# proroklab/gnn_pathplanning

Measured on AMD Instinct MI355X. Metric: agent-steps/sec (policy fwd), higher is better.
Workload: dtype f32 (bf16x3 exact operand split, f32 accumulate); 1 GPU; policy forward (addGSO+forward), 10 agents, 20x20 map GSO, K=3, batch=512 per GPU, eval mode, fp32 GSO resident in HBM; the SAME resident batch every step (inputs are L2 / Infinity-Cache warm by construction); agents=10, taps=3, batch_per_gpu=512, global_batch=512, parallelism=replicas x1

## Files before the change

gnn_pathplanning_amd/_native.py:

```python
import ctypes
import os
import shutil
import subprocess

import torch

_HERE = os.path.dirname(os.path.abspath(__file__))
CSRC = os.path.join(_HERE, 'csrc')
LIB_PATH = os.path.join(_HERE, 'libgnnpp.so')
MEASURE_LIB_PATH = os.path.join(_HERE, 'libgnnpp_measure.so')
VALIDATED_HIPCC = 'HIP version: 7.2.26015-fc0010cf6a'
TOOLCHAIN_STAMP = LIB_PATH + '.toolchain'
H2_UNSAFE_MARK = LIB_PATH + '.split_f16_disabled'
HEADER = os.path.join(os.path.dirname(_HERE), 'include', 'gnnpp.h')
MAPF_DISTANCE_HEADER = os.path.join(os.path.dirname(_HERE), 'include', 'gnnpp_mapf_distance.h')
CASEGEN_HEADER = os.path.join(os.path.dirname(_HERE), 'include', 'gnnpp_casegen.h')
CASEGEN_MAZE_HEADER = os.path.join(os.path.dirname(_HERE), 'include', 'gnnpp_casegen_maze.h')
MAPF_AUDIT_HEADER = os.path.join(os.path.dirname(_HERE), 'include', 'gnnpp_mapf_audit.h')
ROLLOUT_TRACE_HEADER = os.path.join(os.path.dirname(_HERE), 'include', 'gnnpp_rollout_trace.h')
SCHEDULE_DRAW_HEADER = os.path.join(os.path.dirname(_HERE), 'include', 'gnnpp_schedule_draw.h')
ROLLOUT_STREAM_HEADER = os.path.join(os.path.dirname(_HERE), 'include', 'gnnpp_rollout_stream.h')
ROLLOUT_STREAM_TRACE_HEADER = os.path.join(os.path.dirname(_HERE), 'include', 'gnnpp_rollout_stream_trace.h')
HIPCC_FLAGS = ['--offload-arch=gfx950', '-O3', '-std=c++17', '-shared', '-fPIC',
               '-Wno-unused-result']


class GnnppError(RuntimeError):
    pass


OK, ERR_ARG, ERR_UNSUPPORTED, ERR_LAUNCH, ERR_RANGE = 0, -1, -2, -3, -4
PREC_FP32, PREC_FP32_MFMA, PREC_SPLIT_F16 = 0, 1, 2
OBS_C, OBS_HW, FEAT, ACTIONS = 3, 11, 128, 5
MAX_NODES, MAX_ROWS = 100, 112
TUNE_FILTER_GPW, TUNE_FILTER_WAVES, TUNE_FUSED_POLICY, TUNE_FILTER_SPLIT, TUNE_POLICY_FILTER = 1, 2, 6, 7, 9
TUNE_FILTER_SMALL, TUNE_FILTER_SMALL_ROWS, TUNE_FILTER_PIPE_GRID = 10, 11, 12
TUNE_POLICY_CP, TUNE_ENCODER_CP_TILE, TUNE_FILTER_PLANE_ALIAS = 13, 14, 16
TUNE_TRAIN_WGRAD_WGS, TUNE_TRAIN_RUNNING_FUSED, TUNE_ENCODER_ONE_PLANE = 17, 19, 20
ROLLOUT_MAX_AGENTS, ROLLOUT_MAX_TEAM, ROLLOUT_TEAM_MAX_CELLS = 128, 1024, 65536
TIE_LOWEST, TIE_HASHED, TIE_REPLAY, TIE_MT19937 = 0, 1, 2, 3
SCHEDULE_BAD_MOVE, SCHEDULE_BAD_STATE, SCHEDULE_NO_RADIUS = 1, 2, 4
MAPF_NO_PATH, MAPF_BAD_CASE = 1, 2
MAPF_MAX_SIDE, MAPF_MAX_STEPS, MAPF_TEAM_MAX_SIDE, MAPF_TEAM_MAX_STEPS = 64, 1024, 256, 2048
MAPF_DIST_UNREACHABLE, MAPF_DIST_INVALID = -1, -2
MAPF_ORDER_INDEX, MAPF_ORDER_LONGEST_FIRST, MAPF_ORDER_SHORTEST_FIRST, MAPF_ORDER_HASHED = 0, 1, 2, 3
CASEGEN_OK, CASEGEN_TOO_SMALL = 0, 1
MAPF_AUDIT_CHUNK = 32
MAPF_AUDIT_CLASS_STATE, MAPF_AUDIT_CLASS_VERTEX, MAPF_AUDIT_CLASS_MOVE, MAPF_AUDIT_CLASS_SWAP = 0, 1, 2, 3
MAPF_AUDIT_STATE, MAPF_AUDIT_VERTEX, MAPF_AUDIT_MOVE, MAPF_AUDIT_SWAP = 1, 2, 4, 8
MAPF_AUDIT_BAD_START, MAPF_AUDIT_NOT_AT_GOAL, MAPF_AUDIT_SKIPPED = 16, 32, 64
TUNE_FILTER_ABLATE, TUNE_ENCODER_STOP = 3, 4
TUNE_POLICY_CP_TEAM = 21
PRECISIONS = {'fp32': PREC_FP32, 'fp32_mfma': PREC_FP32_MFMA, 'split_f16': PREC_SPLIT_F16}


def precision_code(p):
    if isinstance(p, str):
        if p not in PRECISIONS:
            raise GnnppError('unknown precision %r (one of %s)' % (p, sorted(PRECISIONS)))
        p = PRECISIONS[p]
    else:
        p = int(p)
        if p not in (PREC_FP32, PREC_FP32_MFMA, PREC_SPLIT_F16):
            raise GnnppError('unknown precision code %d' % p)
    if p == PREC_SPLIT_F16 and os.path.exists(H2_UNSAFE_MARK):
        raise GnnppError("precision 'split_f16' is disabled in this build: the ISA hipcc generated for the opt-in "
                         "split-f16 encoder failed the weight-ring check (%s); the default 'fp32' and 'fp32_mfma' "
                         "are unaffected" % open(H2_UNSAFE_MARK).read().strip()[:200])
    return p


def _sources():
    return [os.path.join(CSRC, f) for f in sorted(os.listdir(CSRC))] + [HEADER, MAPF_DISTANCE_HEADER, CASEGEN_HEADER,
                                                                          MAPF_AUDIT_HEADER, ROLLOUT_TRACE_HEADER,
                                                                          SCHEDULE_DRAW_HEADER, ROLLOUT_STREAM_HEADER,
                                                                          CASEGEN_MAZE_HEADER, ROLLOUT_STREAM_TRACE_HEADER]


def build(force=False, verbose=False, measure=False):
    out = MEASURE_LIB_PATH if measure else LIB_PATH
    if (not force and os.path.exists(out)
            and os.path.getmtime(out) >= max(os.path.getmtime(s) for s in _sources())):
        return out
    hipcc = shutil.which('hipcc') or '/opt/rocm/bin/hipcc'
    if not os.path.exists(hipcc):
        raise GnnppError('hipcc not found: libgnnpp.so cannot be built on this machine')
    tmp = os.path.join(_HERE, 'build', 'measure' if measure else 'product')
    os.makedirs(tmp, exist_ok=True)
    tmp_lib = os.path.join(tmp, 'libgnnpp.so')
    cmd = [hipcc] + HIPCC_FLAGS + (['-DGNNPP_MEASURE'] if measure else []) + \
          ['-save-temps', os.path.join(CSRC, 'gnnpp_api.hip'), '-o', tmp_lib]
    if verbose:
        print(' '.join(cmd))
    subprocess.check_call(cmd, cwd=tmp)
    isa = os.path.join(tmp, 'gnnpp_api-hip-amdgcn-amd-amdhsa-gfx950.s')
    h2_errors = check_ring_isa(isa, verbose=verbose)
    if not measure:
        if h2_errors:
            with open(H2_UNSAFE_MARK, 'w') as f:
                f.write('; '.join(h2_errors))
        elif os.path.exists(H2_UNSAFE_MARK):
            os.remove(H2_UNSAFE_MARK)
    if not measure:
        try:
            ver = subprocess.check_output([hipcc, '--version'], stderr=subprocess.STDOUT).decode().splitlines()[0].strip()
        except (OSError, subprocess.CalledProcessError, IndexError):
            ver = 'unknown'
        with open(TOOLCHAIN_STAMP, 'w') as f:
            f.write(ver + '\n')
    for f in os.listdir(tmp):
        if f != os.path.basename(isa) and f != 'libgnnpp.so':
            os.remove(os.path.join(tmp, f))
    os.replace(tmp_lib, out)
    return out


RING_KERNELS = (('encoder_kernel_b3ILb0ELi3ELb0E', 294, 0), ('encoder_kernel_b3ILb1ELi2ELb0E', 342, 32),
                ('encoder_kernel_b3ILb1ELi3ELb0E', 366, 32), ('encoder_kernel_b3ILb1ELi4ELb0E', 390, 32),
                ('encoder_kernel_b3ILb1ELi2ELb1ELi0E', 342, 32), ('encoder_kernel_b3ILb1ELi3ELb1ELi0E', 366, 32),
                ('encoder_kernel_b3ILb1ELi4ELb1ELi0E', 390, 32), ('encoder_kernel_b3ILb0ELi3ELb1ELi0E', 294, 0))
RING_KERNELS_TEAM = (('encoder_kernel_b3ILb1ELi2ELb1ELi10E', 342, 32), ('encoder_kernel_b3ILb1ELi3ELb1ELi10E', 366, 32),
                     ('encoder_kernel_b3ILb1ELi4ELb1ELi10E', 390, 32))
RING_KERNELS_OPTIONAL = (('encoder_kernel_h2ILb0ELi3E', 196, 0), ('encoder_kernel_h2ILb1ELi2E', 228, 32),
                         ('encoder_kernel_h2ILb1ELi3E', 244, 32), ('encoder_kernel_h2ILb1ELi4E', 260, 32))


def check_ring_isa(isa_path, verbose=False):
    import importlib.util
    spec = importlib.util.spec_from_file_location(
        'gnnpp_check_ring_isa', os.path.join(os.path.dirname(_HERE), 'tools', 'check_ring_isa.py'))
    mod = importlib.util.module_from_spec(spec)
    spec.loader.exec_module(mod)
    optional_errors = []
    for kern, items, scratch in RING_KERNELS + RING_KERNELS_TEAM + RING_KERNELS_OPTIONAL:
        errors, stats, meta = mod.check(isa_path, kern, scratch)
# ... 467 lines not shown
```

gnn_pathplanning_amd/csrc/encoder_kernel_b3.hip:

```cpp
#include <utility>

#include "gnnpp_common.h"

namespace gnnpp {

constexpr int kb_L1 = 0, kb_L2 = 54, kb_L3 = 108, kb_L4 = 162, kb_FC = 270, kb_END = 294;
constexpr int kb_FILT = kb_END;

constexpr int kB3Frag = 1024;
constexpr int kB3Region = 25 * 3 * kB3Frag;
constexpr int kB3Obs2 = kObsFloatsLds * 4;
constexpr int kB3L2out = 0, kB3L3out = 24 * kB3Frag, kB3L4out = 48 * kB3Frag;
constexpr int kB3Table = kB3Region;
constexpr int kB3TableBytes = EncLayout::kBssFloats * 4 + 16;
constexpr int kB3TableBytesFused = 5120;
constexpr int kB3SsmOff = 776 * 4;
constexpr size_t kB3Smem = kB3Region + kB3TableBytes;
constexpr size_t kB3SmemFused = kB3Region + kB3TableBytesFused;
static_assert(2 * kObsFloatsLds * 4 <= kB3Region && kB3SsmOff + 16 * 17 * 4 <= kB3TableBytesFused &&
              2 * kB3SmemFused <= (size_t)kLdsBytes, "b3 LDS map");
constexpr int kPkChan = 73;
constexpr int kPkAgent = 231;
constexpr int kPkBytes = kTileAgents * kPkAgent * 4;
constexpr int kB3ForcePlanes = 256;
constexpr int kL0Held = 2;
static_assert(kPkChan >= kPadHW * kPadHW / 2 && kPkAgent >= 3 * kPkChan && (kPkAgent & 1) && kPkBytes % 16 == 0 &&
              kPkBytes <= 2 * kObsFloatsLds * 4, "packed pixel image");
constexpr int kB3ZBytes = 16 * kZs * 4;
constexpr int kB3PRow = 3 * 256 + 32;
constexpr int kB3PBytes = 16 * kB3PRow;
constexpr int kB3POff = 2 * kB3ZBytes;
static_assert(kB3POff + kPolicyTapsMax * kB3PBytes + 4 * 16 * 8 * 4 <= kB3Region, "fused tail fits R");
constexpr size_t policy_sim_occ_bytes_b3() {
    return (size_t)kB3POff - 8 * kMaxAgents * sizeof(int) - kGsoSmemBytes;
}

struct WStreamB {
    const float* seg[6];
    int lane_bytes;
};

__device__ __forceinline__ const float* ring_item_ptr(const WStreamB& ws, int idx) {
    if (idx < kb_L2) return ws.seg[0] + (idx - kb_L1) * EncLayout::kHItem;
    if (idx < kb_L3) return ws.seg[1] + (idx - kb_L2) * EncLayout::kHItem;
    if (idx < kb_L4) return ws.seg[2] + (idx - kb_L3) * EncLayout::kHItem;
    if (idx < kb_FC) return ws.seg[3] + (idx - kb_L4) * EncLayout::kHItem;
    if (idx < kb_FILT) return ws.seg[4] + (idx - kb_FC) * EncLayout::kHItem;
    const int j = idx - kb_FILT, pl = j % 3, ml = (j / 3) & 1, kb = (j / 6) & 3, tap = j / 24;
    return ws.seg[5] + tap * (8 * 4 * 768) + ml * (4 * 768) + kb * 768 + pl * 256;
}

template <int IT, int NKB, int H, int W, int NMT, int NSLOT, class PosFn, bool PRELOAD, int CH = NSLOT>
__device__ __forceinline__ void b3_tap_mfma(const v4f* in, const v4f* Pin, const v8b (&A)[NMT][3],
                                            v4f (&acc)[NSLOT][NMT], int lane) {
    constexpr int kb = IT / 9, tap = IT % 9;
    constexpr int dy = tap / 3 - 1, dx = tap % 3 - 1;
#pragma unroll
    for (int j0 = 0; j0 < NSLOT; j0 += CH) {
        v8b B[CH][3];
#pragma unroll
        for (int jj = 0; jj < CH; ++jj) {
            const int j = j0 + jj;
            int y = 0, x = 0;
            const bool used = j < NSLOT && PosFn::get(j, y, x);
            const int iy = y + dy, ix = x + dx;
            if (used && iy >= 0 && iy < H && ix >= 0 && ix < W) {
                const int o = ((iy * W + ix) * NKB + kb) * 3;
#pragma unroll
                for (int p = 0; p < 3; ++p) B[jj][p] = as_b8(PRELOAD ? Pin[o + p] : in[(o + p) * 64 + lane]);
            }
        }
#pragma unroll
        for (int term = 0; term < kB3Terms; ++term) {
#pragma unroll
            for (int jj = 0; jj < CH; ++jj) {
                const int j = j0 + jj;
                int y = 0, x = 0;
                const bool used = j < NSLOT && PosFn::get(j, y, x);
                const int iy = y + dy, ix = x + dx;
                if (used && iy >= 0 && iy < H && ix >= 0 && ix < W) {
                    const bool fresh = term == 0 && first_step_of_slot<H, W, PosFn>(IT, j);
#pragma unroll
                    for (int m = 0; m < NMT; ++m)
                        acc[j][m] = mfma16b(A[m][b3_term_a(term)], B[jj][b3_term_b(term)],
                                            fresh ? vzero() : acc[j][m]);
                }
            }
        }
    }
}

template <int IT, int CHI, int NKB, int H, int W, int NSLOT, int CH, class PosFn>
__device__ __forceinline__ void b3_load_chunk(const v4f* in, v4f (&B)[CH][3], int lane) {
    constexpr int kb = IT / 9, tap = IT % 9;
    constexpr int dy = tap / 3 - 1, dx = tap % 3 - 1;
#pragma unroll
    for (int jj = 0; jj < CH; ++jj) {
        const int j = CHI * CH + jj;
        int y = 0, x = 0;
        const bool used = j < NSLOT && PosFn::get(j, y, x);
        const int iy = y + dy, ix = x + dx;
        if (used && iy >= 0 && iy < H && ix >= 0 && ix < W) {
            const int o = ((iy * W + ix) * NKB + kb) * 3;
#pragma unroll
            for (int p = 0; p < 3; ++p) B[jj][p] = in[(o + p) * 64 + lane];
        }
    }
// ... 383 lines not shown
    unsigned d[DEPTH + 1][7];
    v4f acc[2][2];
    v4f run[2];
    auto request = [&](unsigned (&dd)[7], int H) {
        const int win = wave + 4 * (H >> 1);
        const int wy = win / 5, wx = win - wy * 5;
        const unsigned* base = obsw + (2 * wy + (H & 1)) * (kPadHW / 2) + wx;
        dd[0] = base[adr[0]];
        dd[4] = base[adr[0] + 7];
        dd[1] = base[adr[1]];
        dd[2] = base[adr[2]];
        dd[3] = base[adr[3]];
        dd[5] = base[adr[4]];
        dd[6] = base[adr[4] + 1];
    };
    auto compute = [&](const unsigned (&dd)[7], auto oxc, v4f (&ac)[2]) {
        constexpr int ox = decltype(oxc)::value;
        const v4u bhv = {__builtin_amdgcn_perm(dd[1], dd[0], selA[ox]),
                         __builtin_amdgcn_perm(dd[3], dd[2], ox ? 0x07060302u : 0x05040100u),
                         __builtin_amdgcn_perm(dd[4], dd[3], selC[ox]),
                         __builtin_amdgcn_perm(dd[6], dd[5], selD[ox])};
        const v8b Bh = __builtin_bit_cast(v8b, bhv);
#pragma unroll
        for (int p = 2; p >= 0; --p)
#pragma unroll
            for (int i = 0; i < 2; ++i) ac[i] = mfma16b(A0[i][p], Bh, p == 2 ? vzero() : ac[i]);
    };
    auto epilogue = [&](const v4f (&ac)[2], int P) {
#pragma unroll
        for (int i = 0; i < 2; ++i) {
            run[i] = (P & 3) == 0 ? ac[i] : vmax(run[i], ac[i]);
            if ((P & 3) == 3) {
                run[i] = vfma(run[i], sc[i], sh[i]);
#pragma unroll
                for (int c = 0; c < 4; ++c) run[i][c] = b3_relu_clamp(run[i][c]);
            }
        }
#if defined(__HIP_DEVICE_COMPILE__)
        asm volatile("" : "+v"(run[0]), "+v"(run[1]));
#endif
    };
    auto window_done = [&](auto wic) {
        constexpr int wi = decltype(wic)::value;
        if constexpr (wi < NHELD) {
            res[wi][0] = run[0];
            res[wi][1] = run[1];
        } else {
            const int win = wave + 4 * wi;
            v4f pl[3];
            b3_split8_clamped(run[0], run[1], pl);
            b3_store_window<CP>(smem, g, win, lane, pl);
        }
    };
    auto prologue = [&](auto p0c, auto p1c, auto kc) {
        constexpr int H = decltype(p0c)::value / 2 + decltype(kc)::value;
        if constexpr (H < decltype(p1c)::value / 2) request(d[H % (DEPTH + 1)], H);
    };
    auto body = [&](auto p0c, auto p1c, auto kc) {
        constexpr int P0 = decltype(p0c)::value, P1 = decltype(p1c)::value, P = P0 + decltype(kc)::value, H = P >> 1;
        if constexpr ((P & 1) == 0 && H + DEPTH < P1 / 2) request(d[(H + DEPTH) % (DEPTH + 1)], H + DEPTH);
        __builtin_amdgcn_sched_barrier(0);
        compute(d[H % (DEPTH + 1)], std::integral_constant<int, (P & 1)>{}, acc[P & 1]);
        if constexpr (P > P0) {
            epilogue(acc[(P - 1) & 1], P - 1);
            if constexpr (((P - 1) & 3) == 3) window_done(std::integral_constant<int, ((P - 1) >> 2)>{});
        }
        __builtin_amdgcn_sched_barrier(0);
        if constexpr (P == P1 - 1) {
            epilogue(acc[P & 1], P);
            window_done(std::integral_constant<int, (P >> 2)>{});
        }
    };
    auto stream = [&](auto p0c, auto p1c) {
        constexpr int N = decltype(p1c)::value - decltype(p0c)::value;
        auto pro = [&](auto... ks) { (prologue(p0c, p1c, ks), ...); };
        auto run_all = [&](auto... ks) { (body(p0c, p1c, ks), ...); };
        [&]<int... K>(std::integer_sequence<int, K...>) { pro(std::integral_constant<int, K>{}...); }(
            std::make_integer_sequence<int, DEPTH>{});
        [&]<int... K>(std::integer_sequence<int, K...>) { run_all(std::integral_constant<int, K>{}...); }(
            std::make_integer_sequence<int, N>{});
    };
    stream(std::integral_constant<int, 0>{}, std::integral_constant<int, 24>{});
    if (wave == 0) stream(std::integral_constant<int, 24>{}, std::integral_constant<int, 28>{});
}

__host__ __device__ __forceinline__ constexpr int cp_ring_item_at(int NA, int i, int s) {
    int first = -1, cnt = 0;
    for (int k = 0; k < 6; ++k)
        if (k * NA / 6 == i) { if (first < 0) first = k; ++cnt; }
    if (cnt == 0 || s % (6 / cnt) != 0 || s / (6 / cnt) >= cnt) return -1;
    return first + s / (6 / cnt);
}
template <class Load, class Hook>
__device__ __forceinline__ void cp_unit(const v8b (&A)[2][3], const v4f (&B)[3], v4f& c0, v4f& c1, Load&& load, Hook&& hook) {
#define GNNPP_CP_M(T, ACC, MI)                                                                          \
    ACC = mfma16b(A[MI][b3_term_a(T)], as_b8(B[b3_term_b(T)]), ACC);                                   \
    __builtin_amdgcn_sched_barrier(0);
#define GNNPP_CP_H(S)                                                                                   \
    hook(std::integral_constant<int, S>{});                                                             \
    __builtin_amdgcn_sched_barrier(0);
    GNNPP_CP_M(0, c0, 0)
    load(0);
    __builtin_amdgcn_sched_barrier(0);
    GNNPP_CP_M(0, c1, 1)
    load(1);
    __builtin_amdgcn_sched_barrier(0);
    GNNPP_CP_M(1, c0, 0)
    load(2);
    __builtin_amdgcn_sched_barrier(0);
    GNNPP_CP_M(1, c1, 1)
    GNNPP_CP_H(0)
    GNNPP_CP_M(2, c0, 0)
    GNNPP_CP_H(1)
    GNNPP_CP_M(2, c1, 1)
    GNNPP_CP_H(2)
    GNNPP_CP_M(3, c0, 0)
    GNNPP_CP_H(3)
    GNNPP_CP_M(3, c1, 1)
    GNNPP_CP_H(4)
    GNNPP_CP_M(4, c0, 0)
    GNNPP_CP_H(5)
    GNNPP_CP_M(4, c1, 1)
    GNNPP_CP_M(5, c0, 0)
    GNNPP_CP_M(5, c1, 1)
#undef GNNPP_CP_H
#undef GNNPP_CP_M
}
template <int BASE, bool FRESH, bool LAST, bool ORDERED, class Load, class Refill>
__device__ __forceinline__ void cp_unit_direct(v4f (&ring)[kRingH], const v4f (&B)[3], v4f& c0, v4f& c1, Load&& load,
                                               Refill&& refill) {
#define GNNPP_CP_M(T, ACC, MI)                                                                          \
    if constexpr (FRESH && T == 0) ring_mfma16b_first(ring, BASE + 3 * MI + b3_term_a(T), B[b3_term_b(T)], ACC);   \
    else ring_mfma16b(ring, BASE + 3 * MI + b3_term_a(T), B[b3_term_b(T)], ACC);                       \
    __builtin_amdgcn_sched_barrier(0);
#define GNNPP_CP_R(K)                                                                                   \
    if constexpr (LAST && !ORDERED) { refill(std::integral_constant<int, K>{}); __builtin_amdgcn_sched_barrier(0); }
    GNNPP_CP_M(0, c0, 0)
    load(0);
    __builtin_amdgcn_sched_barrier(0);
    GNNPP_CP_M(0, c1, 1)
    load(1);
    __builtin_amdgcn_sched_barrier(0);
    GNNPP_CP_M(1, c0, 0)
    load(2);
    __builtin_amdgcn_sched_barrier(0);
    GNNPP_CP_M(1, c1, 1)
    GNNPP_CP_R(2)
    GNNPP_CP_M(2, c0, 0)
    GNNPP_CP_R(5)
    GNNPP_CP_M(2, c1, 1)
    GNNPP_CP_M(3, c0, 0)
    GNNPP_CP_M(3, c1, 1)
    GNNPP_CP_M(4, c0, 0)
    GNNPP_CP_R(1)
    GNNPP_CP_M(4, c1, 1)
    GNNPP_CP_R(4)
    GNNPP_CP_M(5, c0, 0)
    GNNPP_CP_R(0)
    GNNPP_CP_M(5, c1, 1)
    GNNPP_CP_R(3)
    if constexpr (LAST && ORDERED) {
        [&]<int... K>(std::integer_sequence<int, K...>) { (refill(std::integral_constant<int, K>{}), ...); }(
            std::make_integer_sequence<int, 6>{});
        __builtin_amdgcn_sched_barrier(0);
    }
#undef GNNPP_CP_R
// ... 630 lines not shown
#pragma unroll
            for (int k = 0; k < RT; ++k) {
                const unsigned w = tid + k * kThreads;
                if ((int)w < n_rows) {
                    const unsigned ag = w / kRowsPerAgent, rem = w - ag * kRowsPerAgent;
                    const unsigned ch = rem / 11u, y = rem - ch * 11u;
                    unsigned* const dst = obsw + ag * kPkAgent + ch * kPkChan + (y + 1) * (kPadHW / 2);
                    dst[0] = px[k][0] & 0xffff0000u;
#pragma unroll
                    for (int c = 1; c < kPadHW / 2; ++c)
                        dst[c] = __builtin_amdgcn_perm(px[k][2 * c], px[k][2 * c - 1], 0x07060302u);
                }
            }
        } else {
            constexpr int NV4 = (kTileAgents * kObsFloats + 3) / 4 + 1;
            constexpr int PER = (NV4 + kThreads - 1) / kThreads;
            constexpr unsigned AS = kAgentStride, CS = kPadHW * kPadHW;
            const int shift = (int)((reinterpret_cast<uintptr_t>(src) >> 2) & 3);
            const float* src4 = src - shift;
            const long floats_left = (long)(M - agent0) * kObsFloats + shift;
            const bool head_ok = shift == 0 || agent0 > 0;
            v4f v[PER];
#pragma unroll
            for (int k = 0; k < PER; ++k) {
                const int idx = tid + k * kThreads;
                const int e0 = 4 * idx - shift;
                if (head_ok && 4L * idx + 4 <= floats_left && e0 < valid) {
                    v[k] = *reinterpret_cast<const v4f*>(src4 + 4 * idx);
                } else {
#pragma unroll
                    for (int c = 0; c < 4; ++c) v[k][c] = src[min(max(e0 + c, 0), valid - 1)];
                }
            }
            for (int i = tid; i < 2 * kObsFloatsLds / 4; i += kThreads) R4[i] = vzero();
            __syncthreads();
            const unsigned dump = 2 * kObsFloatsLds + lane;
#pragma unroll
            for (int k = 0; k < PER; ++k) {
                const int e0 = (tid + k * kThreads) * 4 - shift;
                const unsigned es = (unsigned)max(e0, 0);
                const unsigned ag = __umul24(es, 46223u) >> 24;
                const unsigned rem = es - __umul24(ag, (unsigned)kObsFloats);
                const unsigned ch = __umul24(rem, 543u) >> 16;
                const int r0 = (int)(rem - __umul24(ch, 121u)) + min(e0, 0);
                const unsigned base = __umul24(ag, AS) + __umul24(ch, CS) + 13u;
                const unsigned wrapped = base + (ch == 2u ? AS - 2 * CS : CS);
                unsigned w1[4], w2[4];
                const v4u vb = __builtin_bit_cast(v4u, v[k]);
                const bool inexact = ((vb[0] | vb[1] | vb[2] | vb[3]) & 0xffffu) != 0u;
                const bool any_l = __ballot(inexact) != 0ull;
                if (!any_l) {
                    w1[0] = vb[0] >> 16; w1[1] = vb[1] >> 16; w1[2] = vb[2] >> 16; w1[3] = vb[3] >> 16;
                } else {
#pragma unroll
                    for (int c2 = 0; c2 < 2; ++c2) {
                        unsigned h, m, l;
                        b3_split2(v[k][2 * c2], v[k][2 * c2 + 1], h, m, l);
                        w1[2 * c2] = __builtin_amdgcn_perm(m, h, 0x05040100u);
                        w1[2 * c2 + 1] = __builtin_amdgcn_perm(m, h, 0x07060302u);
                        w2[2 * c2] = l & 0xffffu;
                        w2[2 * c2 + 1] = l >> 16;
                    }
                }
#pragma unroll
                for (int c = 0; c < 4; ++c) {
                    const int e = e0 + c;
                    int r = r0 + c;
                    const bool wrap = r >= 121;
                    r = wrap ? r - 121 : r;
                    const unsigned y = __umul24((unsigned)r & 0xffu, 745u) >> 13;
                    const unsigned o = (wrap ? wrapped : base) + (unsigned)r + y;
                    const bool ok = e >= 0 && e < valid;
                    obsw[ok ? o : dump] = w1[c];
                    if (any_l) obsw[ok ? o + kObsFloatsLds : dump] = w2[c];
                }
            }
        }
    }
    __syncthreads();
    if (GNNPP_STOP_AT(stop, 1)) return;
    if (!pt.with_sim) GNNPP_STAMP(blockIdx.x, 0, tid == 0);

    {
        if (one_plane) {
            v4f res[kL0Held][2];
            b3_l0_stream<CP>(pk, obsw, sstab, gnnpp_smem, geom, res, wave, lane);
            __syncthreads();
#pragma unroll
            for (int wi = 0; wi < kL0Held; ++wi) {
                const int win = wave + 4 * wi;
                v4f pl[3];
                b3_split8_clamped(res[wi][0], res[wi][1], pl);
                b3_store_window<CP>(gnnpp_smem, geom, win, lane, pl);
            }
        } else {
            b3_l0_generic<CP>(pk, obsw, sstab, gnnpp_smem, geom, wave, lane);
        }
    }
    __syncthreads();
    if (GNNPP_STOP_AT(stop, 2)) return;
    if (!pt.with_sim) GNNPP_STAMP(blockIdx.x, 1, tid == 0);

    if constexpr (CP) {
        cp_layer1<END, NFIX>(ws, ring, gnnpp_smem, sstab, geom, wave, lane, tid);
    } else {
        v4f acc[7][2];
        constexpr int CH1 = 2;
        v4f Bb[2][CH1][3];
        auto layer1 = [&](auto wc) {
            using P = PosL1H<decltype(wc)::value>;
            b3_load_chunk<0, 0, 1, 5, 5, 7, CH1, P>(R4, Bb[0], lane);
            b3_stream_steps<END, kb_L1, 2>(ws, ring, [&](auto itc, const v8b (&A)[2][3]) {
                b3_step_pipelined<decltype(itc)::value, 9, 1, 5, 5, 2, 7, CH1, P>(R4, Bb, A, acc, lane);
            }, std::make_integer_sequence<int, 9>{});
        };
        switch (wave) {
            case 0: layer1(std::integral_constant<int, 0>{}); break;
            case 1: layer1(std::integral_constant<int, 1>{}); break;
            case 2: layer1(std::integral_constant<int, 2>{}); break;
            default: layer1(std::integral_constant<int, 3>{}); break;
        }
        __syncthreads();
        v4f sc[2], sh[2];
        load_ss(sstab + EncLayout::kBssL1, 32, 0, q, sc[0], sh[0]);
        load_ss(sstab + EncLayout::kBssL1, 32, 1, q, sc[1], sh[1]);
#pragma unroll
        for (int j = 0; j < 7; ++j) {
            const int p = wave + 4 * j;
            if (p < 25) {
                v4f pl[3];
                b3_split8_clamped(vrelu_clamp(vfma(acc[j][0], sc[0], sh[0])), vrelu_clamp(vfma(acc[j][1], sc[1], sh[1])), pl);
#pragma unroll
                for (int pp = 0; pp < 3; ++pp) R4[(p * 3 + pp) * 64 + lane] = pl[pp];
            }
        }
    }
    __syncthreads();
    if (GNNPP_STOP_AT(stop, 3)) return;
    if (!pt.with_sim) GNNPP_STAMP(blockIdx.x, 2, tid == 0);

    if constexpr (CP) {
        cp_layer2<END, NFIX>(ws, ring, gnnpp_smem, sstab, geom, wave, lane);
    } else {
        const int mp = wave & 1, pair = wave >> 1;
        v4f acc[8][2];
        constexpr int CH2 = 2;
        v4f Bb[2][CH2][3];
        auto layer2 = [&](auto pc) {
            using P = PosL2H<decltype(pc)::value>;
            b3_load_chunk<0, 0, 1, 5, 5, 8, CH2, P>(R4, Bb[0], lane);
            b3_stream_steps<END, kb_L2, 2>(ws, ring, [&](auto itc, const v8b (&A)[2][3]) {
                b3_step_pipelined<decltype(itc)::value, 9, 1, 5, 5, 2, 8, CH2, P>(R4, Bb, A, acc, lane);
            }, std::make_integer_sequence<int, 9>{});
        };
        switch (pair) {
            case 0: layer2(std::integral_constant<int, 0>{}); break;
            default: layer2(std::integral_constant<int, 1>{}); break;
        }
        v4f sc[2], sh[2];
        load_ss(sstab + EncLayout::kBssL2, 64, 2 * mp, q, sc[0], sh[0]);
        load_ss(sstab + EncLayout::kBssL2, 64, 2 * mp + 1, q, sc[1], sh[1]);
        v4f r[2][2];
#pragma unroll
        for (int wi = 0; wi < 2; ++wi)
#pragma unroll
            for (int m = 0; m < 2; ++m) {
                r[wi][m] = vrelu(vfma(acc[4 * wi][m], sc[m], sh[m]));
// ... 156 lines not shown
#pragma unroll
    for (int tap = 0; tap < KT; ++tap) {
        const char* zr = gnnpp_smem + kB3POff + tap * kB3PBytes + a * kB3PRow + q * 16;
#pragma unroll
        for (int kb = 0; kb < 4; ++kb) {
            __builtin_amdgcn_sched_barrier(kSchedItemMask);
            v8b A[2][3];
#pragma unroll
            for (int m = 0; m < 2; ++m)
#pragma unroll
                for (int p = 0; p < 3; ++p) {
                    const int idx = kb_FILT + ((tap * 4 + kb) * 2 + m) * 3 + p;
                    A[m][p] = as_b8(ring_take_f4<END>(ring, idx));
                    h2_ring_load<END>(ws, ring, idx + kRingH);
                }
            v8b B[3];
#pragma unroll
            for (int p = 0; p < 3; ++p) B[p] = as_b8(*reinterpret_cast<const v4f*>(zr + p * 256 + kb * 64));
#pragma unroll
            for (int term = 0; term < kB3Terms; ++term)
#pragma unroll
                for (int m = 0; m < 2; ++m) {
                    if (term == kB3Terms - 1) fa[m] = mfma16b(A[m][0], B[0], fa[m]);
                    else fc[m] = mfma16b(A[m][b3_term_a(term)], B[b3_term_b(term)], fc[m]);
                }
        }
    }
    GNNPP_STAMP(blockIdx.x, 14, tid == 0);
    float* const yb = reinterpret_cast<float*>(gnnpp_smem + kB3POff + KT * kB3PBytes);
    {
        v4f d = vzero();
#pragma unroll
        for (int m = 0; m < 2; ++m) {
            const int f0 = (2 * wave + m) * 16 + 4 * q;
            const v4f bv = *reinterpret_cast<const v4f*>(hconst + 640 + f0);
            const v4f A5 = a < 5 ? *reinterpret_cast<const v4f*>(hconst + a * 128 + f0) : vzero();
            d = mfma16x4(A5, vrelu((fa[m] + fc[m]) + bv), d);
        }
        if (q < 2) *reinterpret_cast<v4f*>(yb + (wave * 16 + a) * 8 + 4 * q) = d;
    }
    __syncthreads();
    int* const spos = reinterpret_cast<int*>(gnnpp_smem);
    if (wave == 0) {
        v4f d = *reinterpret_cast<const v4f*>(yb + a * 8 + 4 * (q & 1));
#pragma unroll
        for (int w = 1; w < kWaves; ++w) d += *reinterpret_cast<const v4f*>(yb + (w * 16 + a) * 8 + 4 * (q & 1));
        const v4f ab4 = *reinterpret_cast<const v4f*>(hconst + 768 + 4 * (q & 1));
        if (a < pt.N && q < 2) {
            float* dst = pt.logits + ((size_t)a * pt.B + blockIdx.x) * 5;
            float* lds = reinterpret_cast<float*>(spos) + 4 * kMaxAgents + a * 5;
            if (q == 0) {
#pragma unroll
                for (int t = 0; t < 4; ++t) {
                    dst[t] = d[t] + ab4[t];
                    if (pt.with_sim) lds[t] = d[t] + ab4[t];
                }
            } else {
                dst[4] = d[0] + ab4[0];
                if (pt.with_sim) lds[4] = d[0] + ab4[0];
            }
        }
        __builtin_amdgcn_wave_barrier();
    }
    if (!pt.with_sim) return;

    {
        int* red = spos + 2 * kMaxAgents;
        int* goal_l = red + 4 * kMaxAgents;
        char* gso_smem = reinterpret_cast<char*>(goal_l + 2 * kMaxAgents);
        unsigned char* occ = reinterpret_cast<unsigned char*>(gso_smem + kGsoSmemBytes);
        const int b = blockIdx.x;
        GNNPP_STAMP(b, 10, tid == 0);
        const size_t occ_bytes = ((size_t)pt.sim.H * pt.sim.W + 15) & ~(size_t)15;
        unsigned* cellcnt = 2 * occ_bytes <= policy_sim_occ_bytes_b3() ? reinterpret_cast<unsigned*>(occ + occ_bytes)
                                                                       : nullptr;
        sim_tail(pt.sim, b, spos, red, goal_l, gso_smem, occ, tid, kThreads, cellcnt,
                 reinterpret_cast<const float*>(red + 2 * kMaxAgents));
    }
}

std::atomic<int> g_policy_column_packing{1};
#define GNNPP_TUNE_POLICY_CP_TEAM 21
std::atomic<int> g_policy_cp_team{1};
std::atomic<int> g_encoder_one_plane{1};
static int b3_plane_flag() { return g_encoder_one_plane.load(std::memory_order_relaxed) ? 0 : kB3ForcePlanes; }
std::atomic<int> g_encoder_cp_tile{0};

static int encoder_cp_tile(int M) {
    const int knob = g_encoder_cp_tile.load(std::memory_order_relaxed);
    if (knob >= 1 && knob <= kCpMaxAgents) return knob;
    if (knob != 0 || g_policy_column_packing.load(std::memory_order_relaxed) == 0) return 0;
    const int t = (M + 255) / 256;
    return t <= 8 ? t : 0;
}

int encoder_launch_b3(const float* obs, const float* packed, float* feat, int M, hipStream_t st) {
    if (const int tile = encoder_cp_tile(M)) {
        static LdsAttrOnce once_cp;
        set_lds_attr_once(once_cp, reinterpret_cast<const void*>(&encoder_kernel_b3<false, 3, true>), (int)kB3Smem);
        PolicyTail pt{};
        pt.N = tile;
        hipLaunchKernelGGL((encoder_kernel_b3<false, 3, true>), dim3((M + tile - 1) / tile), dim3(kThreads), kB3Smem, st,
                           obs, packed, feat, M, GNNPP_ENCODER_STOP_VALUE | b3_plane_flag(), pt);
        return hipGetLastError() == hipSuccess ? 0 : -3;
    }
    static LdsAttrOnce once;
    set_lds_attr_once(once, reinterpret_cast<const void*>(&encoder_kernel_b3<false, 3>), (int)kB3Smem);
    const int grid = (M + kTileAgents - 1) / kTileAgents;
    hipLaunchKernelGGL((encoder_kernel_b3<false, 3>), dim3(grid), dim3(kThreads), kB3Smem, st, obs, packed, feat, M,
                       GNNPP_ENCODER_STOP_VALUE | b3_plane_flag(), PolicyTail{});
    return hipGetLastError() == hipSuccess ? 0 : -3;
}

template <int KT, bool CP, int NFIX = 0>
static int policy_launch_fused_b3_k(const float* obs, const float* packed, const PolicyTail& pt, hipStream_t st) {
    static LdsAttrOnce once;
    set_lds_attr_once(once, reinterpret_cast<const void*>(&encoder_kernel_b3<true, KT, CP, NFIX>), (int)kB3SmemFused);
    hipLaunchKernelGGL((encoder_kernel_b3<true, KT, CP, NFIX>), dim3(pt.B), dim3(kThreads), kB3SmemFused, st, obs, packed,
                       static_cast<float*>(nullptr), pt.B * pt.N, b3_plane_flag(), pt);
    return hipGetLastError() == hipSuccess ? 0 : -3;
}
template <int KT>
static int policy_launch_fused_b3_form(const float* obs, const float* packed, const PolicyTail& pt, hipStream_t st) {
    if (pt.N > kCpMaxAgents || g_policy_column_packing.load(std::memory_order_relaxed) == 0)
        return policy_launch_fused_b3_k<KT, false>(obs, packed, pt, st);
    if (pt.N == kCpTeamFixed && g_policy_cp_team.load(std::memory_order_relaxed) != 0)
        return policy_launch_fused_b3_k<KT, true, kCpTeamFixed>(obs, packed, pt, st);
    return policy_launch_fused_b3_k<KT, true>(obs, packed, pt, st);
}

int policy_launch_fused_b3(const float* obs, const float* packed, const PolicyTail& pt, int K, hipStream_t st) {
    switch (K) {
        case 2: return policy_launch_fused_b3_form<2>(obs, packed, pt, st);
        case 3: return policy_launch_fused_b3_form<3>(obs, packed, pt, st);
        case 4: return policy_launch_fused_b3_form<4>(obs, packed, pt, st);
        default: return -2;
    }
}

}
```

gnn_pathplanning_amd/csrc/gnnpp_api.hip:

```cpp
#include "../../include/gnnpp.h"
#ifdef GNNPP_MEASURE
#include "gnnpp_measure.h"
#endif

#include "encoder_pack.hip"
#include "encoder_ring_f32.hip"
#include "encoder_kernel_f32.hip"
#include "comm_graph.hip"
#include "rollout_kernels.hip"
#include "rollout_team_kernels.hip"
#include "expert_kernels.hip"
#include "expert_team_kernels.hip"
#include "mapf_kernels.hip"
#include "mapf_team_kernels.hip"
#include "mapf_distance_kernels.hip"
#include "casegen_kernels.hip"
#include "casegen_maze_kernels.hip"
#include "mapf_audit_kernels.hip"
#include "encoder_kernel_h2.hip"
#include "encoder_kernel_b3.hip"
#include "lsigf_kernel.hip"
#include "policy_filter_kernel.hip"
#include "lsigf_small_kernel.hip"
#include "lsigf_team_kernel.hip"
// ... 446 lines not shown
    size_t n = 0;
    for (int i = 0; i < count; ++i)
        if (d[i].batch > 0 && d[i].M > 0 && d[i].N > 0 && d[i].K > 0)
            n += gemm_workspace_floats(d[i].batch, d[i].M, d[i].N, d[i].K);
    return n;
}

int gnnpp_gemm_kmajor_multi(const gnnpp_gemm_desc* d, int count, float* workspace, void* stream) {
    if (!d || count <= 0 || count > kGemmMax) return GNNPP_ERR_ARG;
    GemmTable tb = {};
    for (int i = 0; i < count; ++i) {
        if (!d[i].A || !d[i].B || !d[i].C || d[i].batch <= 0 || d[i].M <= 0 || d[i].N <= 0 || d[i].K <= 0)
            return GNNPP_ERR_ARG;
        GemmOne& g = tb.g[i];
        g.A = d[i].A; g.a_sb = (long)d[i].a_sb; g.a_sm = (long)d[i].a_sm; g.a_sk = (long)d[i].a_sk;
        g.B = d[i].B; g.b_sb = (long)d[i].b_sb; g.b_sk = (long)d[i].b_sk;
        g.C = d[i].C; g.c_sb = (long)d[i].c_sb; g.c_sm = (long)d[i].c_sm;
        g.batch = d[i].batch; g.M = d[i].M; g.N = d[i].N; g.K = d[i].K; g.mask = d[i].mask;
    }
    tb.count = count;
    if (gnnpp_gemm_multi_workspace_floats(d, count) > 0 && !workspace) return GNNPP_ERR_ARG;
    return gemm_multi_launch(tb, workspace, static_cast<hipStream_t>(stream));
}

int gnnpp_linear_fwd(const float* x, const float* W, const float* bias, float* y, int R, int I, int O, int relu,
                     void* stream) {
    if (!x || !W || !y || R <= 0 || I <= 0 || O <= 0) return GNNPP_ERR_ARG;
    if (I % 64 != 0 || ((reinterpret_cast<size_t>(x) | reinterpret_cast<size_t>(W)) & 15)) return GNNPP_ERR_UNSUPPORTED;
    if ((O & 3) == 0 && (reinterpret_cast<size_t>(y) & 15)) return GNNPP_ERR_UNSUPPORTED;
    const int tiles = ((O + 15) / 16) * ((R + 15) / 16);
    hipLaunchKernelGGL(linear_fwd_kernel, dim3((tiles + 3) / 4), dim3(256), 0, static_cast<hipStream_t>(stream), x, W,
                       bias, y, R, I, O, relu);
    return hipGetLastError() == hipSuccess ? GNNPP_OK : GNNPP_ERR_LAUNCH;
}

int gnnpp_policy_loss(const float* logits, const float* target, float* loss, float* dlogits, int B, int N,
                      int C, int logits_sample_major, void* stream) {
    if (!logits || !target || !loss || B <= 0 || N <= 0 || C <= 0 || C > 64) return GNNPP_ERR_ARG;
    hipLaunchKernelGGL(policy_loss_kernel, dim3(1), dim3(1024), 1024 * sizeof(double),
                       static_cast<hipStream_t>(stream), logits, target, loss, dlogits, B, N, C, logits_sample_major);
    return hipGetLastError() == hipSuccess ? GNNPP_OK : GNNPP_ERR_LAUNCH;
}

int gnnpp_adam_step(const gnnpp_adam_tensors* t, float* state, float lr, float beta1, float beta2, float eps,
                    float weight_decay, int tick, void* stream) {
    if (!t || !state || t->count <= 0 || t->count > kAdamTensors) return GNNPP_ERR_ARG;
    hipStream_t st = static_cast<hipStream_t>(stream);
    AdamTable tb = {};
    int blocks = 0;
    for (int i = 0; i < t->count; ++i) {
        if (!t->p[i] || !t->g[i] || !t->m[i] || !t->v[i] || t->numel[i] <= 0) return GNNPP_ERR_ARG;
        tb.p[i] = t->p[i]; tb.g[i] = t->g[i]; tb.m[i] = t->m[i]; tb.v[i] = t->v[i];
        tb.numel[i] = (long)t->numel[i];
        tb.first[i] = blocks;
        blocks += (int)((t->numel[i] + 1023) / 1024);
    }
    tb.first[t->count] = blocks;
    tb.count = t->count;
    hipLaunchKernelGGL(adam_kernel, dim3(blocks), dim3(256), 4 * sizeof(float), st, tb, state, lr, beta1, beta2, eps,
                       weight_decay, tick ? 1 : 0);
    return hipGetLastError() == hipSuccess ? GNNPP_OK : GNNPP_ERR_LAUNCH;
}

#ifdef GNNPP_MEASURE
int gnnpp_measure_read_stamps(unsigned long long* host, int n) {
    if (!host || n <= 0 || n > 1024 * 32) return GNNPP_ERR_ARG;
    return hipMemcpyFromSymbol(host, HIP_SYMBOL(g_stamps), (size_t)n * sizeof(unsigned long long)) == hipSuccess
               ? GNNPP_OK : GNNPP_ERR_LAUNCH;
}
#endif

int gnnpp_get_tuning(int key) {
    switch (key) {
        case GNNPP_TUNE_FILTER_GPW: return g_filter_gpw.load();
        case GNNPP_TUNE_FILTER_WAVES: return g_filter_waves.load();
        case GNNPP_TUNE_FUSED_POLICY: return g_fused_policy.load();
        case GNNPP_TUNE_FILTER_SPLIT: return g_filter_split.load();
        case GNNPP_TUNE_POLICY_FILTER: return g_filter_policy_kernel.load();
        case GNNPP_TUNE_FILTER_SMALL: return g_filter_small_kernel.load();
        case GNNPP_TUNE_FILTER_SMALL_ROWS: return g_filter_small_rows.load();
        case GNNPP_TUNE_FILTER_PIPE_GRID: return g_filter_pipe_grid.load();
        case GNNPP_TUNE_POLICY_CP: return g_policy_column_packing.load();
        case GNNPP_TUNE_POLICY_CP_TEAM: return g_policy_cp_team.load();
        case GNNPP_TUNE_ENCODER_CP_TILE: return g_encoder_cp_tile.load();
        case GNNPP_TUNE_FILTER_PLANE_ALIAS: return g_filter_plane_alias.load();
        case GNNPP_TUNE_TRAIN_WGRAD_WGS: return g_train_wgrad_wgs.load();
        case GNNPP_TUNE_TRAIN_RUNNING_FUSED: return g_train_running_fused.load();
        case GNNPP_TUNE_ENCODER_ONE_PLANE: return g_encoder_one_plane.load();
#ifdef GNNPP_MEASURE
        case GNNPP_TUNE_FILTER_ABLATE: return g_filter_ablate.load();
        case GNNPP_TUNE_ENCODER_STOP: return g_encoder_stop.load();
#endif
        default: return GNNPP_ERR_ARG;
    }
}

int gnnpp_set_tuning(int key, int value) {
    switch (key) {
        case GNNPP_TUNE_FILTER_GPW:
            if (value < 0) return GNNPP_ERR_ARG;
            g_filter_gpw.store(value);
            return GNNPP_OK;
        case GNNPP_TUNE_FUSED_POLICY:
            if (value < 0 || value > 2) return GNNPP_ERR_ARG;
            g_fused_policy.store(value);
            return GNNPP_OK;
        case GNNPP_TUNE_FILTER_WAVES:
            if (value != 0 && value != 8 && value != 16) return GNNPP_ERR_ARG;
            g_filter_waves.store(value);
            return GNNPP_OK;
        case GNNPP_TUNE_FILTER_SPLIT:
            if (value < 0 || value > 7) return GNNPP_ERR_ARG;
            g_filter_split.store(value);
            return GNNPP_OK;
        case GNNPP_TUNE_POLICY_FILTER:
            if (value < 0 || value > 1) return GNNPP_ERR_ARG;
            g_filter_policy_kernel.store(value);
            return GNNPP_OK;
        case GNNPP_TUNE_FILTER_SMALL_ROWS:
            if (value != 0 && value != 32 && value != 48 && value != 64) return GNNPP_ERR_ARG;
            g_filter_small_rows.store(value);
            return GNNPP_OK;
        case GNNPP_TUNE_FILTER_PIPE_GRID:
            if (value < 0 || value > 4096) return GNNPP_ERR_ARG;
            g_filter_pipe_grid.store(value);
            return GNNPP_OK;
        case GNNPP_TUNE_POLICY_CP:
            if (value != 0 && value != 1) return GNNPP_ERR_ARG;
            g_policy_column_packing.store(value);
            return GNNPP_OK;
        case GNNPP_TUNE_POLICY_CP_TEAM:
            if (value != 0 && value != 1) return GNNPP_ERR_ARG;
            g_policy_cp_team.store(value);
            return GNNPP_OK;
        case GNNPP_TUNE_ENCODER_CP_TILE:
            if (value != 0 && value != 16 && (value < 1 || value > 12)) return GNNPP_ERR_ARG;
            g_encoder_cp_tile.store(value);
            return GNNPP_OK;
        case GNNPP_TUNE_FILTER_PLANE_ALIAS:
            if (value < 0 || value > 1) return GNNPP_ERR_ARG;
            g_filter_plane_alias.store(value);
            return GNNPP_OK;
        case GNNPP_TUNE_TRAIN_RUNNING_FUSED:
            if (value < 0 || value > 1) return GNNPP_ERR_ARG;
            g_train_running_fused.store(value);
            return GNNPP_OK;
        case GNNPP_TUNE_ENCODER_ONE_PLANE:
            if (value < 0 || value > 1) return GNNPP_ERR_ARG;
            g_encoder_one_plane.store(value);
            return GNNPP_OK;
        case GNNPP_TUNE_TRAIN_WGRAD_WGS:
            if (value != 0 && (value < 16 || value > 2048)) return GNNPP_ERR_ARG;
            g_train_wgrad_wgs.store(value);
            return GNNPP_OK;
        case GNNPP_TUNE_FILTER_SMALL:
            if (value < 0 || value > 3) return GNNPP_ERR_ARG;
            g_filter_small_kernel.store(value);
            return GNNPP_OK;
#ifdef GNNPP_MEASURE
        case GNNPP_TUNE_ENCODER_STOP:
            if (value < 0 || value > 6) return GNNPP_ERR_ARG;
            g_encoder_stop.store(value);
            return GNNPP_OK;
        case GNNPP_TUNE_FILTER_ABLATE:
            g_filter_ablate.store(value);
            return GNNPP_OK;
#endif
        default:
            return GNNPP_ERR_ARG;
    }
}

int gnnpp_decode_actions(const float* logits, int* actions, int B, int N, void* stream) {
    if (!logits || !actions || B <= 0 || N <= 0) return GNNPP_ERR_ARG;
    return decode_actions_launch(logits, actions, B, N, static_cast<hipStream_t>(stream));
}

static int rollout_common_ok(const gnnpp_rollout* r, int max_agents = GNNPP_ROLLOUT_MAX_TEAM) {
    return r && r->pos && r->B > 0 && r->N > 0 && r->N <= max_agents;
}

static bool rollout_team(const gnnpp_rollout* r) { return r->N > GNNPP_ROLLOUT_MAX_AGENTS; }

int gnnpp_rollout_observe(const gnnpp_rollout* r, void* stream) {
    if (!rollout_common_ok(r) || !r->grid || !r->goal || !r->obs || r->H <= 0 || r->W <= 0)
        return GNNPP_ERR_ARG;
    if (rollout_team(r)) return rollout_team_observe_launch(*r, static_cast<hipStream_t>(stream));
    return rollout_observe_launch(*r, static_cast<hipStream_t>(stream));
}

int gnnpp_rollout_gso(const gnnpp_rollout* r, void* stream) {
    if (!rollout_common_ok(r) || !r->radius || !r->S) return GNNPP_ERR_ARG;
    if (rollout_team(r)) return rollout_team_gso_launch(*r, r->grow != 0, static_cast<hipStream_t>(stream));
    return rollout_gso_launch(*r, static_cast<hipStream_t>(stream));
}

int gnnpp_rollout_lists(const gnnpp_rollout* r, void* lists, size_t lists_bytes, void* stream) {
    if (!rollout_common_ok(r) || !r->radius || !team_lists_block_ok(lists, lists_bytes, r->B, r->N)) return GNNPP_ERR_ARG;
    return rollout_team_lists_launch(*r, r->grow != 0, lists, static_cast<hipStream_t>(stream));
}

int gnnpp_rollout_gso_observe(const gnnpp_rollout* r, void* stream) {
    if (!rollout_common_ok(r) || !r->radius || !r->S || !r->grid || !r->goal || !r->obs || r->H <= 0 || r->W <= 0)
        return GNNPP_ERR_ARG;
    if (rollout_team(r)) return rollout_team_gso_observe_launch(*r, static_cast<hipStream_t>(stream));
    return rollout_gso_observe_launch(*r, static_cast<hipStream_t>(stream));
}

static bool rollout_move_ok(const gnnpp_rollout* r, int max_agents = GNNPP_ROLLOUT_MAX_TEAM) {
    if (!rollout_common_ok(r, max_agents) || !r->grid || !r->goal || (!r->logits && !r->actions) ||
        !r->reached || !r->start_step || !r->end_step || !r->maxstep || !r->flags || !r->stats ||
        r->H <= 0 || r->W <= 0)
        return false;
    if (r->tie_mode == GNNPP_TIE_REPLAY && (!r->choices || r->max_choices <= 0)) return false;
    if (r->tie_mode < 0 || r->tie_mode > 3) return false;
    return !(r->tie_mode == GNNPP_TIE_MT19937 && (!r->rng_words || !r->rng_cursor || r->rng_max <= 0));
// ... 414 lines not shown
```

Before: 107.3 million agent-steps/s.

## Add packed fixed-team L0 conv path ordering columns by window and agent

Adds a specialized first-conv-layer routine for the ten-agent column-packed team encoder. Each MFMA column maps to a (window, agent) pair, operands are gathered straight from the packed pixel image via byte-perm, and output tiles are written to the L1 input rows without the separate per-plane pass and its barrier. It is enabled by default through a new tuning flag and comes with compile-time checks on division tricks, row overlap and the LDS bank-conflict profile, which still shows some conflicts.

```diff
diff --git a/gnn_pathplanning_amd/_native.py b/gnn_pathplanning_amd/_native.py
--- a/gnn_pathplanning_amd/_native.py
+++ b/gnn_pathplanning_amd/_native.py
@@ -51,6 +51,7 @@
 MAPF_AUDIT_BAD_START, MAPF_AUDIT_NOT_AT_GOAL, MAPF_AUDIT_SKIPPED = 16, 32, 64
 TUNE_FILTER_ABLATE, TUNE_ENCODER_STOP = 3, 4
 TUNE_POLICY_CP_TEAM = 21
+TUNE_POLICY_CP_TEAM_L0 = 22
 PRECISIONS = {'fp32': PREC_FP32, 'fp32_mfma': PREC_FP32_MFMA, 'split_f16': PREC_SPLIT_F16}
 
 
diff --git a/gnn_pathplanning_amd/csrc/encoder_kernel_b3.hip b/gnn_pathplanning_amd/csrc/encoder_kernel_b3.hip
--- a/gnn_pathplanning_amd/csrc/encoder_kernel_b3.hip
+++ b/gnn_pathplanning_amd/csrc/encoder_kernel_b3.hip
@@ -23,6 +23,7 @@
 constexpr int kPkAgent = 231;
 constexpr int kPkBytes = kTileAgents * kPkAgent * 4;
 constexpr int kB3ForcePlanes = 256;
+constexpr int kB3L0ByAgent = 512;
 constexpr int kL0Held = 2;
 static_assert(kPkChan >= kPadHW * kPadHW / 2 && kPkAgent >= 3 * kPkChan && (kPkAgent & 1) && kPkBytes % 16 == 0 &&
               kPkBytes <= 2 * kObsFloatsLds * 4, "packed pixel image");
@@ -572,6 +573,171 @@
     };
     stream(std::integral_constant<int, 0>{}, std::integral_constant<int, 24>{});
     if (wave == 0) stream(std::integral_constant<int, 24>{}, std::integral_constant<int, 28>{});
+}
+
+__host__ __device__ constexpr int cp_l0f_window(int c) { return c < 25 * kCpTeamFixed ? c / kCpTeamFixed : 0; }
+__host__ __device__ constexpr int cp_l0f_agent(int c) {
+    return c < 25 * kCpTeamFixed ? c % kCpTeamFixed : c - 25 * kCpTeamFixed + kCpTeamFixed;
+}
+__host__ __device__ constexpr int cp_l0f_base(int c) {
+    return cp_l0f_agent(c) * kPkAgent + (2 * (cp_l0f_window(c) / 5)) * (kPadHW / 2) + cp_l0f_window(c) % 5;
+}
+__host__ __device__ constexpr int cp_l0f_role(int q, int k) {
+    return q < 3 ? q * kPkChan + (k == 0 ? 0 : k < 3 ? 1 : k == 3 ? 6 : 12) : k < 3 ? k * kPkChan + 13 : 0;
+}
+__host__ __device__ constexpr bool cp_l0f_divisions_ok() {
+    for (int c = 0; c < 256; ++c)
+        if (((c * 205) >> 11) != c / 10) return false;
+    for (int w = 0; w <= 25; ++w)
+        if (((w * 52) >> 8) != w / 5) return false;
+    return true;
+}
+struct CpL0fBanks { int worst, doubled_max, doubled_all; };
+__host__ __device__ constexpr CpL0fBanks cp_l0f_banks() {
+    CpL0fBanks r = {0, 0, 0};
+    for (int t = 0; t < 16; ++t) {
+        int base[16] = {};
+        for (int j = 0; j < 16; ++j) base[j] = cp_l0f_base(16 * t + j);
+        int doubled = 0;
+        for (int acc = 0; acc < 7; ++acc) {
+            const int k = acc < 2 ? 0 : acc > 4 ? 4 : acc - 1, plus = acc == 1 ? 7 : acc == 6 ? 1 : 0;
+            int cnt[64] = {};
+            for (int l = 0; l < 64; ++l) ++cnt[(base[l & 15] + cp_l0f_role(l >> 4, k) + plus) & 63];
+            for (int b = 0; b < 64; ++b) {
+                if (cnt[b] > r.worst) r.worst = cnt[b];
+                if (cnt[b] > 1) doubled += cnt[b] - 1;
+            }
+        }
+        if (doubled > r.doubled_max) r.doubled_max = doubled;
+        r.doubled_all += 2 * doubled;
+    }
+    return r;
+}
+constexpr CpL0fBanks kCpL0fBanks = cp_l0f_banks();
+__host__ __device__ constexpr bool cp_l0f_rows_clear_pixels() {
+    constexpr int T1 = (25 * kCpTeamFixed + 15) >> 4, l1in = kB3Region - (T1 + 1) * kCpRow;
+    return T1 == 16 && l1in >= kPkBytes && 16 * T1 - 25 * kCpTeamFixed <= kTileAgents - kCpTeamFixed;
+}
+
+template <int NFIX>
+__device__ __forceinline__ void b3_l0_stream_fixed(const float* __restrict__ pk, const float* sstab, char* smem,
+                                                   int wave, int lane) {
+    static_assert(NFIX == kCpTeamFixed && kCpTeamFixed == 10, "the column order and its divisions are written for ten agents");
+    static_assert(cp_l0f_divisions_ok(), "c / 10 and w / 5 as multiply-shift");
+    static_assert(cp_l0f_rows_clear_pixels(), "every tile is stored while other waves still read pixels");
+    static_assert(kCpL0fBanks.worst == 3 && kCpL0fBanks.doubled_max == 115 && kCpL0fBanks.doubled_all == 3030,
+                  "LDS banks of the packed L0's reads (not conflict-free: see above)");
+    constexpr int DEPTH = 2;
+    constexpr int l1in = kB3Region - 17 * kCpRow;
+    const int j = lane & 15, q = lane >> 4;
+    v8b A0[2][3];
+#pragma unroll
+    for (int i = 0; i < 2; ++i)
+#pragma unroll
+        for (int p = 0; p < 3; ++p)
+            A0[i][p] = as_b8(*reinterpret_cast<const v4f*>(pk + EncLayout::kB0 + ((i * 3 + p) * 64 + lane) * 4));
+    int role[5];
+    role[0] = q < 3 ? q * kPkChan : 13;
+    role[1] = q < 3 ? q * kPkChan + 1 : kPkChan + 13;
+    role[2] = q < 3 ? q * kPkChan + 1 : 2 * kPkChan + 13;
+    role[3] = q < 3 ? q * kPkChan + 6 : 0;
+    role[4] = q < 3 ? q * kPkChan + 12 : 0;
+    int adr[4][5];
+#pragma unroll
+    for (int ti = 0; ti < 4; ++ti) {
+        const int c = 16 * (wave + 4 * ti) + j;
+        const bool real = c < 25 * NFIX;
+        const int w = real ? (c * 205) >> 11 : 0, n = real ? c - w * NFIX : c - 24 * NFIX;
+        const int wy = (w * 52) >> 8, wx = w - 5 * wy;
+        const int base = n * kPkAgent + wy * (2 * (kPadHW / 2)) + wx;
+#pragma unroll
+        for (int k = 0; k < 5; ++k) adr[ti][k] = 4 * (base + role[k]);
+#if defined(__HIP_DEVICE_COMPILE__)
+        asm volatile("" : "+v"(adr[ti][0]), "+v"(adr[ti][1]), "+v"(adr[ti][2]), "+v"(adr[ti][3]), "+v"(adr[ti][4]));
+#endif
+    }
+    unsigned selA[2], selC[2], selD[2];
+    selA[0] = q < 3 ? 0x03020100u : 0x05040100u;  selA[1] = q < 3 ? 0x05040302u : 0x07060302u;
+    selC[0] = q < 3 ? 0x05040302u : 0x01000100u;  selC[1] = q < 3 ? 0x07060504u : 0x03020302u;
+    selD[0] = q < 3 ? 0x03020100u : 0x01000100u;  selD[1] = q < 3 ? 0x05040302u : 0x03020302u;
+#if defined(__HIP_DEVICE_COMPILE__)
+    asm volatile("" : "+v"(selA[0]), "+v"(selA[1]), "+v"(selC[0]), "+v"(selC[1]), "+v"(selD[0]), "+v"(selD[1]));
+#endif
+    v4f sc[2], sh[2];
+    load_ss(sstab + EncLayout::kBssL0, 32, 0, q, sc[0], sh[0]);
+    load_ss(sstab + EncLayout::kBssL0, 32, 1, q, sc[1], sh[1]);
+    unsigned d[DEPTH + 1][7];
+    v4f acc[2][2];
+    v4f run[2];
+    auto request = [&](unsigned (&dd)[7], auto hc) {
+        constexpr int ti = decltype(hc)::value >> 1, oy = (decltype(hc)::value & 1) * (kPadHW / 2);
+        auto at = [&](int k) { return reinterpret_cast<const unsigned*>(smem + adr[ti][k]); };
+        dd[0] = at(0)[oy];
+        dd[4] = at(0)[oy + 7];
+        dd[1] = at(1)[oy];
+        dd[2] = at(2)[oy];
+        dd[3] = at(3)[oy];
+        dd[5] = at(4)[oy];
+        dd[6] = at(4)[oy + 1];
+    };
+    auto compute = [&](const unsigned (&dd)[7], auto oxc, v4f (&ac)[2]) {
+        constexpr int ox = decltype(oxc)::value;
+        const v4u bhv = {__builtin_amdgcn_perm(dd[1], dd[0], selA[ox]),
+                         __builtin_amdgcn_perm(dd[3], dd[2], ox ? 0x07060302u : 0x05040100u),
+                         __builtin_amdgcn_perm(dd[4], dd[3], selC[ox]),
+                         __builtin_amdgcn_perm(dd[6], dd[5], selD[ox])};
+        const v8b Bh = __builtin_bit_cast(v8b, bhv);
+#pragma unroll
+        for (int p = 2; p >= 0; --p)
+#pragma unroll
+            for (int i = 0; i < 2; ++i) ac[i] = mfma16b(A0[i][p], Bh, p == 2 ? vzero() : ac[i]);
+    };
+    auto epilogue = [&](const v4f (&ac)[2], int P) {
+#pragma unroll
+        for (int i = 0; i < 2; ++i) {
+            run[i] = (P & 3) == 0 ? ac[i] : vmax(run[i], ac[i]);
+            if ((P & 3) == 3) {
+                run[i] = vfma(run[i], sc[i], sh[i]);
+#pragma unroll
+                for (int c = 0; c < 4; ++c) run[i][c] = b3_relu_clamp(run[i][c]);
+            }
+        }
+#if defined(__HIP_DEVICE_COMPILE__)
+        asm volatile("" : "+v"(run[0]), "+v"(run[1]));
+#endif
+    };
+    auto tile_done = [&](auto tic) {
+        const int t = wave + 4 * decltype(tic)::value;
+        v4f pl[3];
+        b3_split8_clamped(run[0], run[1], pl);
+        if (16 * t + j < 25 * NFIX) {
+            char* const dst = smem + l1in + t * kCpRow + lane * 16;
+#pragma unroll
+            for (int p = 0; p < 3; ++p) *reinterpret_cast<v4f*>(dst + p * kB3Frag) = pl[p];
+        }
+    };
+    constexpr int NP = 16;
+    auto body = [&](auto kc) {
+        constexpr int P = decltype(kc)::value, H = P >> 1;
+        if constexpr ((P & 1) == 0 && H + DEPTH < NP / 2)
+            request(d[(H + DEPTH) % (DEPTH + 1)], std::integral_constant<int, H + DEPTH>{});
+        __builtin_amdgcn_sched_barrier(0);
+        compute(d[H % (DEPTH + 1)], std::integral_constant<int, (P & 1)>{}, acc[P & 1]);
+        if constexpr (P > 0) {
+            epilogue(acc[(P - 1) & 1], P - 1);
+            if constexpr (((P - 1) & 3) == 3) tile_done(std::integral_constant<int, ((P - 1) >> 2)>{});
+        }
+        __builtin_amdgcn_sched_barrier(0);
+        if constexpr (P == NP - 1) {
+            epilogue(acc[P & 1], P);
+            tile_done(std::integral_constant<int, (P >> 2)>{});
+        }
+    };
+    [&]<int... K>(std::integer_sequence<int, K...>) {
+        (request(d[K % (DEPTH + 1)], std::integral_constant<int, K>{}), ...);
+    }(std::make_integer_sequence<int, DEPTH>{});
+    [&]<int... K>(std::integer_sequence<int, K...>) { (body(std::integral_constant<int, K>{}), ...); }(
+        std::make_integer_sequence<int, NP>{});
 }
 
 __host__ __device__ __forceinline__ constexpr int cp_ring_item_at(int NA, int i, int s) {
@@ -1368,7 +1534,11 @@
     if (!pt.with_sim) GNNPP_STAMP(blockIdx.x, 0, tid == 0);
 
     {
-        if (one_plane) {
+        bool packed_l0 = false;
+        if constexpr (CP && NFIX == kCpTeamFixed) packed_l0 = one_plane && (stop_flags & kB3L0ByAgent) == 0;
+        if (packed_l0) {
+            if constexpr (CP && NFIX == kCpTeamFixed) b3_l0_stream_fixed<NFIX>(pk, sstab, gnnpp_smem, wave, lane);
+        } else if (one_plane) {
             v4f res[kL0Held][2];
             b3_l0_stream<CP>(pk, obsw, sstab, gnnpp_smem, geom, res, wave, lane);
             __syncthreads();
@@ -1691,6 +1861,9 @@
 std::atomic<int> g_policy_column_packing{1};
 #define GNNPP_TUNE_POLICY_CP_TEAM 21
 std::atomic<int> g_policy_cp_team{1};
+#define GNNPP_TUNE_POLICY_CP_TEAM_L0 22
+std::atomic<int> g_policy_cp_team_l0{1};
+static int b3_l0_flag() { return g_policy_cp_team_l0.load(std::memory_order_relaxed) ? 0 : kB3L0ByAgent; }
 std::atomic<int> g_encoder_one_plane{1};
 static int b3_plane_flag() { return g_encoder_one_plane.load(std::memory_order_relaxed) ? 0 : kB3ForcePlanes; }
 std::atomic<int> g_encoder_cp_tile{0};
@@ -1726,7 +1899,7 @@
     static LdsAttrOnce once;
     set_lds_attr_once(once, reinterpret_cast<const void*>(&encoder_kernel_b3<true, KT, CP, NFIX>), (int)kB3SmemFused);
     hipLaunchKernelGGL((encoder_kernel_b3<true, KT, CP, NFIX>), dim3(pt.B), dim3(kThreads), kB3SmemFused, st, obs, packed,
-                       static_cast<float*>(nullptr), pt.B * pt.N, b3_plane_flag(), pt);
+                       static_cast<float*>(nullptr), pt.B * pt.N, b3_plane_flag() | b3_l0_flag(), pt);
     return hipGetLastError() == hipSuccess ? 0 : -3;
 }
 template <int KT>
diff --git a/gnn_pathplanning_amd/csrc/gnnpp_api.hip b/gnn_pathplanning_amd/csrc/gnnpp_api.hip
--- a/gnn_pathplanning_amd/csrc/gnnpp_api.hip
+++ b/gnn_pathplanning_amd/csrc/gnnpp_api.hip
@@ -552,6 +552,7 @@
         case GNNPP_TUNE_FILTER_PIPE_GRID: return g_filter_pipe_grid.load();
         case GNNPP_TUNE_POLICY_CP: return g_policy_column_packing.load();
         case GNNPP_TUNE_POLICY_CP_TEAM: return g_policy_cp_team.load();
+        case GNNPP_TUNE_POLICY_CP_TEAM_L0: return g_policy_cp_team_l0.load();
         case GNNPP_TUNE_ENCODER_CP_TILE: return g_encoder_cp_tile.load();
         case GNNPP_TUNE_FILTER_PLANE_ALIAS: return g_filter_plane_alias.load();
         case GNNPP_TUNE_TRAIN_WGRAD_WGS: return g_train_wgrad_wgs.load();
@@ -602,6 +603,10 @@
         case GNNPP_TUNE_POLICY_CP_TEAM:
             if (value != 0 && value != 1) return GNNPP_ERR_ARG;
             g_policy_cp_team.store(value);
+            return GNNPP_OK;
+        case GNNPP_TUNE_POLICY_CP_TEAM_L0:
+            if (value != 0 && value != 1) return GNNPP_ERR_ARG;
+            g_policy_cp_team_l0.store(value);
             return GNNPP_OK;
         case GNNPP_TUNE_ENCODER_CP_TILE:
             if (value != 0 && value != 16 && (value < 1 || value > 12)) return GNNPP_ERR_ARG;
```

Result: faster. 112.1 million agent-steps/s, median of 6 (+4.4%).
